# XuyangBai/D3Feat.pytorch

Measured on AMD Instinct MI355X. Metric: fragment-pairs/sec (fwd+bwd) on 3DMatch-shaped pairs, higher is better.
Workload: dtype f32

## Files before the change

### d3feat.pytorch_amd/_native.py

```python
import ctypes as C
import os
import subprocess

_PKG_DIR = os.path.dirname(os.path.abspath(__file__))
_REPO = os.path.dirname(_PKG_DIR)
LIB_PATH = os.path.join(_PKG_DIR, "libd3feat_hip.so")
CSRC = os.path.join(_PKG_DIR, "csrc")
SOURCES = ["radius_neighbors.hip", "grid_subsample.hip", "kpconv.hip", "kpconv_fused.hip", "kpconv_aggregate.hip", "kpconv_small.hip", "kpconv_deform.hip", "pool.hip", "detection.hip", "loss.hip",
           "reverse_table.hip", "kpconv_dx_gather.hip", "matching.hip", "elementwise.hip", "batchnorm.hip", "linear.hip", "gemm_epilogue.hip", "optimizer.hip", "misc.hip",
           "registration.hip", "nearest_pairs.hip", "icp.hip", "normals.hip", "augment.hip", "posegraph.hip", "tsdf.hip", "tsdf_integrate.hip", "tsdf_mesh.hip", "tsdf_sparse.hip", "odometry.hip", "tsdf_raycast.hip",
           "tsdf_mesh_sparse.hip"]

_vp, _i, _f, _sz = C.c_void_p, C.c_int, C.c_float, C.c_size_t
_d = C.c_double


class Tunables(C.Structure):
    _fields_ = [("atb_task_us", C.c_int32), ("atb_form", C.c_int32), ("atb_first_form_wgs", C.c_int32),
                ("match_wgs", C.c_int32), ("agg_through_lds", C.c_int32), ("atb_pipe", C.c_int32), ("xw_rows", C.c_int32), ("xw_split", C.c_int32),
                ("rowgemm_wide", C.c_int32), ("rowgemm_rt", C.c_int32), ("reserved", C.c_int32 * 6)]


class AtbProblem(C.Structure):
    _fields_ = [("x", _vp), ("grad_out", _vp), ("grad_w", _vp), ("N", C.c_int32), ("Cin", C.c_int32),
# ... 84 lines not shown
    "d3f_kpconv_packs_supports": (_i, [_i, _i, _i, _i, _i]),
    "d3f_kpconv_saves_wf": (_i, [_i, _i, _i, _i]),
    "d3f_kpconv_backward": (_i, [_vp, _i, _vp, _i, _vp, _i, _vp, _i, _vp, _i, _vp, _i, _f, _vp, _vp, _vp, _vp, _i,
                                 _vp, _vp, _vp, _sz, _vp]),
    "d3f_kpconv_grad_input_supported": (_i, [_i, _i, _i, _i]),
    "d3f_kpconv_aggregate": (_i, [_vp, _i, _vp, _i, _vp, _i, _vp, _i, _vp, _i, _f, _vp, _vp, _vp, _vp, _vp, _sz, _vp]),
    "d3f_kpconv_aggregate_modes": (_i, [_vp, _i, _vp, _i, _vp, _i, _vp, _i, _vp, _i, _f, _i, _vp, _vp, _vp]),
    "d3f_kpconv_grad_input_modes": (_i, [_vp, _i, _vp, _i, _vp, _i, _i, _vp, _i, _f, _i, _vp, _vp, _vp]),
    "d3f_kpconv_grad_input": (_i, [_vp, _i, _vp, _i, _vp, _i, _vp, _i, _vp, _i, _f, _vp, _vp, _i, _vp, _vp, _sz, _vp]),
    "d3f_kpconv_aggregate_transposed_supported": (_i, [_i, _i]),
    "d3f_kpconv_aggregate_transposed": (_i, [_vp, _i, _i, _i, _vp, _i, _f, _vp, _vp, _i, _vp, _vp]),
    "d3f_reverse_table_ws_bytes": (_sz, [_i, _i, _i]),
    "d3f_reverse_table_build": (_i, [_vp, _i, _i, _i, _vp, _vp, _vp, _sz, _vp]),
    "d3f_kpconv_grad_input_gather_supported": (_i, [_i, _i, _i]),
    "d3f_kpconv_grad_input_gather": (_i, [_vp, _i, _vp, _i, _vp, _vp, _vp, _i, _f, _vp, _vp, _i, _vp, _i, _i, _f, _vp, _vp, _vp,
                                          _vp, _vp]),
    "d3f_reverse_table_filter": (_i, [_vp, _i, _vp, _vp, _i, _vp, _i, _f, _vp, _vp, _vp]),
    "d3f_linear_grad_weight_supported": (_i, [_i, _i, _i]),
    "d3f_linear_fused_supported": (_i, [_i, _i, _i]),
    "d3f_linear_bias_act_forward": (_i, [_vp, _vp, _i, _i, _i, _vp, _vp, _vp, _f, _vp, _vp, _i, _vp]),
    "d3f_linear_pair_supported": (_i, [_i, _i, _i, _i]),
    "d3f_linear_pair_bias_act_forward": (_i, [_vp, _vp, _i, _vp, _vp, _i, _i, _i, _vp, _vp, _vp, _vp, _f, _vp, _vp, _i, _vp]),
    "d3f_linear_grad_input": (_i, [_vp, _vp, _i, _i, _i, _vp, _vp, _vp]),
    "d3f_linear_grad_weight_ws_bytes": (_sz, [_i, _i, _i]),
    "d3f_linear_grad_weight": (_i, [_vp, _vp, _i, _i, _i, _vp, _vp, _sz, _vp]),
    "d3f_linear_grad_weight_bias": (_i, [_vp, _vp, _i, _i, _i, _vp, _vp, _sz, _vp, _i, _i, _vp, _vp, _vp]),
    "d3f_permute_kpconv_weights": (_i, [_vp, _vp, _vp, _vp, _vp, _i, _vp]),
    "d3f_gemm_epilogue_supported": (_i, [_i, _i, _i, _i, _i]),
    "d3f_gemm_epilogue_ws_bytes": (_sz, [_i, _i, _i]),
    "d3f_gemm_epilogue": (_i, [_vp, _i, _vp, _i, _i, _i, _i, _i, _i, _vp, _vp, _vp, _i, _vp, _f, _vp, _i, _vp, _i, _vp, _sz,
                               _vp]),
    "d3f_bias_act_backward_blocks": (_i, [_i, _i]),
    "d3f_bias_act_backward_partial": (_i, [_vp, _vp, _f, _i, _i, _vp, _vp, _vp, _sz, _vp]),
    "d3f_bias_sum": (_i, [_vp, _i, _i, _vp, _vp, _vp]),
    "d3f_max_pool_forward": (_i, [_vp, _i, _i, _vp, _i, _i, _vp, _vp, _vp, _vp, _vp, _i, _i, _vp]),
    "d3f_max_pool_backward": (_i, [_vp, _vp, _i, _i, _i, _vp, _i, _vp]),
    "d3f_closest_pool_forward": (_i, [_vp, _i, _i, _vp, _i, _i, _vp, _i, _vp, _vp, _vp]),
    "d3f_closest_pool_backward": (_i, [_vp, _i, _vp, _i, _i, _i, _i, _vp, _i, _vp]),
    "d3f_bias_act_forward": (_i, [_vp, _vp, _vp, _vp, _f, _i, _i, _vp, _vp, _i, _vp, _vp, _i, _i, _vp]),
    "d3f_bias_act_backward_ws_bytes": (_sz, [_i, _i]),
    "d3f_bias_act_backward": (_i, [_vp, _vp, _f, _i, _i, _vp, _vp, _vp, _i, _vp, _vp, _sz, _vp]),
    "d3f_global_max": (_i, [_vp, _sz, _vp, _vp, _sz, _vp]),
    "d3f_global_max_rows": (_i, [_vp, _i, _i, _vp, _i, _vp, _vp, _sz, _vp]),
    "d3f_global_max_groups": (_i, [_vp, _i, _i, _vp, _i, _i, _vp, _vp, _sz, _vp]),
    "d3f_detection_scores_aux_floats": (_i, [_i]),
    "d3f_detection_scores_forward": (_i, [_vp, _i, _i, _vp, _i, _vp, _i, _vp, _vp, _vp, _vp, _i, _i, _vp]),
# ... 245 lines not shown
```

### d3feat.pytorch_amd/csrc/linear.hip

```cpp
#include <math.h>

#include <vector>

#include "kpconv_tile.hpp"

namespace d3f {

void* kpconv_timing_open(int which, hipStream_t stream, int Nq, int Ns, int H, int Cin, int Cout, int K);
void kpconv_timing_close(void* rec, hipStream_t stream);

template <int TI, int TJ, int U>
__global__ __launch_bounds__(256, 4) void atb_partial_kernel(const float* __restrict__ A, const float* __restrict__ B,
                                                             const float* __restrict__ row_div, int R, int M, int N,
                                                             int rows_per_wg, float* __restrict__ part) {
  typedef typename VecT<TI>::type VA;
  typedef typename VecT<TJ>::type VB;
  constexpr int HALVES = (TI * TJ >= 16) ? 2 : 1, TH = TI / HALVES;
  __shared__ float red[3][TH * TJ * 256];
  const int lane = threadIdx.x & 63, wave = threadIdx.x >> 6;
  const int li = lane & 15, lk = lane >> 4;
  const int nbj = N / (16 * TJ);
  const int m0 = (blockIdx.y / nbj) * 16 * TI, n0 = (blockIdx.y % nbj) * 16 * TJ;
  const int r0 = blockIdx.x * rows_per_wg, r1 = min(R, r0 + rows_per_wg);
  const float* ap = A + m0 + TI * li;
// ... 1059 lines not shown
bool rowgemm_pair_supported(int N, int K1, int K2, int M) {
  return N >= 4096 && ((M == 128 && K1 == 32 && K2 == 64) || (M == 64 && K1 == 16 && K2 == 32));
}

static int rowgemm_pair_launch(const float* X1, const float* W1, int K1, const float* X2, const float* W2, int K2, int N,
                               int M, const float* b1, const float* b2, const float* b3, const float* b4, float slope,
                               float* Y, float* zinit, int zn, hipStream_t stream) {
  if (!rowgemm_pair_supported(N, K1, K2, M)) return D3F_EINVAL;
  const int rw = tunables().rowgemm_wide;
  const bool wide = rw == 2 || (rw == 0 && N >= 65536);
#define D3F_RGPT(MBW, CS, KA, KB)                                                                                      \
  rowgemm_rt_kernel<MBW, CS, KA, KB><<<cdiv(N, 32 * (4 / CS)), 256, 0, stream>>>(X1, W1, X2, W2, N, b1, nullptr, b2, b3, \
                                                                                  b4, slope, Y, zinit, zn)
  if (M == 128) {
    if (wide) D3F_RGPT(4, 2, 2, 4); else D3F_RGPT(2, 4, 2, 4);
  } else {
    if (wide) D3F_RGPT(4, 1, 1, 2); else D3F_RGPT(2, 2, 1, 2);
  }
#undef D3F_RGPT
  D3F_LAUNCH_CHECK();
  return D3F_OK;
}

}

extern "C" {

int d3f_linear_grad_weight_supported(int N, int Cin, int Cout) { return d3f::atb_supported(N, Cout, Cin) ? 1 : 0; }

size_t d3f_linear_grad_weight_ws_bytes(int N, int Cin, int Cout) { return d3f::atb_ws_bytes(N, Cout, Cin); }

int d3f_linear_grad_weight(const float* x, const float* grad_out, int N, int Cin, int Cout, float* grad_w, void* ws,
                           size_t ws_bytes, void* stream) {
  if (!x || !grad_out || !grad_w || !ws || !d3f::atb_supported(N, Cout, Cin)) return D3F_EINVAL;
  if (ws_bytes < d3f::atb_ws_bytes(N, Cout, Cin)) return D3F_EWORKSPACE;
  return d3f::atb_splitk(grad_out, x, nullptr, N, Cout, Cin, grad_w, ws, (hipStream_t)stream);
}

int d3f_linear_grad_weight_bias(const float* x, const float* grad_out, int N, int Cin, int Cout, float* grad_w, void* ws,
                                size_t ws_bytes, const float* bias_part, int bias_blocks, int bias_cols,
                                float* grad_bias, float* grad_bias2, void* stream) {
  if (!x || !grad_out || !grad_w || !ws || !d3f::atb_supported(N, Cout, Cin)) return D3F_EINVAL;
  if (!bias_part || !grad_bias || bias_blocks < 1 || bias_cols < 1) return D3F_EINVAL;
  if (ws_bytes < d3f::atb_ws_bytes(N, Cout, Cin)) return D3F_EWORKSPACE;
  return d3f::atb_splitk_bias(grad_out, x, nullptr, N, Cout, Cin, grad_w, ws, (hipStream_t)stream, 0, bias_part,
                              bias_blocks, bias_cols, grad_bias, grad_bias2);
// ... 41 lines not shown
  return d3f::rowgemm_pair_supported(N, Cin1, Cin2, Cout) ? 1 : 0;
}

int d3f_linear_pair_bias_act_forward(const float* x1, const float* w1, int Cin1, const float* x2, const float* w2, int Cin2,
                                     int N, int Cout, const float* bias1, const float* bias2, const float* bias3,
                                     const float* bias4, float slope, float* out, float* zero_init, int zero_n,
                                     void* stream) {
  if (!x1 || !w1 || !x2 || !w2 || !out || !d3f::rowgemm_pair_supported(N, Cin1, Cin2, Cout) || (zero_init && zero_n < 1))
    return D3F_EINVAL;
  return d3f::rowgemm_pair_launch(x1, w1, Cin1, x2, w2, Cin2, N, Cout, bias1, bias2, bias3, bias4, slope, out, zero_init,
                                  zero_n, (hipStream_t)stream);
}

int d3f_linear_grad_input(const float* grad_out, const float* weight, int N, int Cin, int Cout, const float* add,
                          float* grad_x, void* stream) {
  if (!grad_out || !weight || !grad_x || !d3f::rowgemm_supported(N, Cout, Cin)) return D3F_EINVAL;
  if (add)
    return d3f::rowgemm_launch<false, true>(grad_out, weight, N, Cout, Cin, nullptr, add, nullptr, 1.0f, grad_x,
                                            nullptr, 0, (hipStream_t)stream);
  return d3f::rowgemm_launch<false, false>(grad_out, weight, N, Cout, Cin, nullptr, nullptr, nullptr, 1.0f, grad_x,
                                           nullptr, 0, (hipStream_t)stream);
}

}
```

### d3feat.pytorch_amd/ops.py

```python
import collections
import numpy as np
import ctypes
import threading

import torch

from . import _native

ORDER_REFERENCE = 0
ORDER_FIRST_SEEN = 1


def _stream():
    return torch.cuda.current_stream().cuda_stream


_PROFILER = None


def set_profiler(p):
    global _PROFILER
    _PROFILER = p


# ... 869 lines not shown
    def collect(self):
        self.closed = True
        g, self.tensor = self.tensor, None
        return g


class _GradTapFn(torch.autograd.Function):

    @staticmethod
    def forward(ctx, x, holder):
        ctx.holder = holder
        return x.view_as(x)

    @staticmethod
    def backward(ctx, g):
        return (None if ctx.holder.deposit(g) else g), None


def grad_tap(x, holder):
    return _GradTapFn.apply(x, holder) if holder is not None else x


def _add_deposited(holder, go, weight):
    c = holder.collect() if holder is not None else None
    if c is None:
        return torch.mm(go, weight)
    if c.is_contiguous() and c.dtype == go.dtype and c.shape == (go.shape[0], weight.shape[1]):
        if _WG_GROUP is not None:
            N, Cout, Cin = int(go.shape[0]), int(go.shape[1]), int(weight.shape[1])
            L = _native.lib()
            if go.is_contiguous() and weight.is_contiguous() and L.d3f_linear_fused_supported(N, Cin, Cout):
                gx = torch.empty_like(c)
                _native.check(L.d3f_linear_grad_input(_p(go), _p(weight), N, Cin, Cout, _p(c), _p(gx), _stream()),
                              "d3f_linear_grad_input")
                return gx
            return torch.addmm(c, go, weight)
        return c.addmm_(go, weight)
    return torch.mm(go, weight).add_(c)


GEMM_NT, GEMM_NN = 0, 1


def _al16(*ts):
    return all(t is None or t.data_ptr() % 16 == 0 for t in ts)


# ... 68 lines not shown
                                     b2 is not None and ctx.needs_input_grad[4], Cout, x.device)
        with _region("linear_fused_fwd[N=%d,Cin=%d,Cout=%d]" % (N, Cin, Cout), 4 * N * (Cin + Cout) + 4 * Cin * Cout):
            _native.check(L.d3f_linear_bias_act_forward(_p(x), _p(weight), N, Cin, Cout, _p(b1), _p(add), _p(b2),
                                                        float(slope), _p(out), _p(gbuf), nb * Cout, _stream()),
                          "d3f_linear_bias_act_forward")
        ctx.save_for_backward(x, weight, out)
        ctx.gbuf = gbuf
        ctx.gw_slot = _grad_slot(weight)
        ctx.slope = float(slope)
        ctx.has = (b1 is not None, add is not None, b2 is not None)
        return out

    @staticmethod
    def backward(ctx, grad_out):
        x, weight, out = ctx.saved_tensors
        L = _native.lib()
        N, Cin, Cout = int(x.shape[0]), int(x.shape[1]), int(weight.shape[0])
        go = grad_out.contiguous()
        want1 = ctx.has[0] and ctx.needs_input_grad[2]
        want2 = ctx.has[2] and ctx.needs_input_grad[4]
        g1, g2, first, second, pre = _bias_grad_rows(ctx, want1, want2, Cout, go.device)
        atb = ctx.needs_input_grad[1] and bool(L.d3f_linear_grad_weight_supported(N, Cin, Cout))
        bias_part, bias_blocks = None, 0
        if ctx.slope == 1.0 and not (want1 or want2):
            gm = go
        else:
            gm = go if ctx.slope == 1.0 else torch.empty_like(go)
            bias_part, bias_blocks = _epilogue_backward(go, out, ctx.slope, N, Cout, gm if ctx.slope != 1.0 else None,
                                                        first, second, pre, None, atb)
        gx = gw = None
        if ctx.needs_input_grad[0]:
            gx = torch.empty_like(x)
            c = ctx.holder.collect() if ctx.holder is not None else None
            if c is not None and not (c.is_contiguous() and c.shape == gx.shape and c.dtype == gx.dtype):
                c = c.contiguous().float().reshape(gx.shape)
            with _region("linear_dx[N=%d,Cin=%d,Cout=%d]" % (N, Cin, Cout), 4 * N * (Cin + Cout) + 4 * Cin * Cout):
                _native.check(L.d3f_linear_grad_input(_p(gm), _p(weight), N, Cin, Cout, _p(c), _p(gx), _stream()),
                              "d3f_linear_grad_input")
            if ctx.dep is not None and ctx.dep.deposit(gx):
                gx = None
        if ctx.needs_input_grad[1]:
            gw = _grad_target(ctx.gw_slot, weight)
            _weight_grad(x, gm, N, Cin, Cout, gw, atb, bias_part, bias_blocks, first, second)
        return (gx, _adoptable(gw, ctx.gw_slot), g1, gm if ctx.has[1] and ctx.needs_input_grad[3] else None, g2,
                None, None, None)


class _LinearPairBiasActFn(torch.autograd.Function):

    @staticmethod
    def forward(ctx, x1, w1, b1a, b1b, x2, w2, b2a, b2b, slope, deposit2=None):
        L = _native.lib()
        ctx.dep2 = deposit2
        N, C1, C2, Cout = int(x1.shape[0]), int(x1.shape[1]), int(x2.shape[1]), int(w1.shape[0])
        out = torch.empty((N, Cout), dtype=torch.float32, device=x1.device)
        ctx.want = tuple(b is not None and ctx.needs_input_grad[i] for b, i in ((b1a, 2), (b1b, 3), (b2a, 6), (b2b, 7)))
        gbuf, nb = _bias_grad_buffer(any(ctx.want), any(ctx.want), Cout, x1.device)
        with _region("linear_pair_fwd[N=%d,Cin=%d|%d,Cout=%d]" % (N, C1, C2, Cout),
                     4 * N * (C1 + C2 + Cout) + 4 * (C1 + C2) * Cout):
            _native.check(L.d3f_linear_pair_bias_act_forward(_p(x1), _p(w1), C1, _p(x2), _p(w2), C2, N, Cout, _p(b1a),
                                                             _p(b1b), _p(b2a), _p(b2b), float(slope), _p(out), _p(gbuf),
                                                             nb * Cout, _stream()), "d3f_linear_pair_bias_act_forward")
        ctx.save_for_backward(x1, w1, x2, w2, out)
        ctx.gbuf, ctx.slope = gbuf, float(slope)
        ctx.slots = (_grad_slot(w1), _grad_slot(w2))
        return out

    @staticmethod
    def backward(ctx, grad_out):
        x1, w1, x2, w2, out = ctx.saved_tensors
        L = _native.lib()
        N, C1, C2, Cout = int(x1.shape[0]), int(x1.shape[1]), int(x2.shape[1]), int(w1.shape[0])
        go = grad_out.contiguous()
        first, second, _, _, pre = _bias_grad_rows(ctx, any(ctx.want), any(ctx.want), Cout, go.device)
        need_w1, need_w2 = ctx.needs_input_grad[1], ctx.needs_input_grad[5]
        fold = need_w1 and need_w2 and _WG_GROUP is not None
        gm = torch.empty_like(go) if ctx.slope != 1.0 else go
        bias_part, bias_blocks = None, 0
        if ctx.slope != 1.0 or first is not None:
            bias_part, bias_blocks = _epilogue_backward(go, out, ctx.slope, N, Cout, gm if ctx.slope != 1.0 else None, first,
                                                        second, pre, None, fold and first is not None)
        third = fourth = None
        if first is not None:
            third, fourth = torch.empty_like(first), torch.empty_like(first)
        gx1 = gx2 = None
        if ctx.needs_input_grad[0]:
            gx1 = torch.empty_like(x1)
            _native.check(L.d3f_linear_grad_input(_p(gm), _p(w1), N, C1, Cout, None, _p(gx1), _stream()),
                          "d3f_linear_grad_input")
        if ctx.needs_input_grad[4]:
            gx2 = torch.empty_like(x2)
            _native.check(L.d3f_linear_grad_input(_p(gm), _p(w2), N, C2, Cout, None, _p(gx2), _stream()),
                          "d3f_linear_grad_input")
            if ctx.dep2 is not None and ctx.dep2.deposit(gx2):
                gx2 = None
        gw1 = gw2 = None
        if need_w1:
            gw1 = _grad_target(ctx.slots[0], w1)
            _weight_grad(x1, gm, N, C1, Cout, gw1, True, bias_part, bias_blocks, first, second)
        if need_w2:
            gw2 = _grad_target(ctx.slots[1], w2)
            _weight_grad(x2, gm, N, C2, Cout, gw2, True, bias_part, bias_blocks, third, fourth)
        if first is not None and bias_part is None:
            third.copy_(first)
            fourth.copy_(first)
        g = [first if ctx.want[0] else None, second if ctx.want[1] else None, third if ctx.want[2] else None,
             fourth if ctx.want[3] else None]
        return (gx1, _adoptable(gw1, ctx.slots[0]), g[0], g[1], gx2, _adoptable(gw2, ctx.slots[1]), g[2], g[3],
                None, None)


def linear_pair_supported(N, C1, C2, Cout, *tensors):
    for t in tensors:
        if not (t.is_cuda and t.dtype == torch.float32 and t.is_contiguous() and t.data_ptr() % 16 == 0):
            return False
    L = _native.lib()
    N, C1, C2, Cout = int(N), int(C1), int(C2), int(Cout)
    return bool(L.d3f_linear_pair_supported(N, C1, C2, Cout)) and bool(L.d3f_linear_fused_supported(N, C1, Cout)) \
        and bool(L.d3f_linear_fused_supported(N, C2, Cout))


def linear_pair_bias_act(x1, w1, b1a, b1b, x2, w2, b2a, b2b, slope=0.1, grad_deposit2=None):
    f = _opt_f32
    if not linear_pair_supported(x1.shape[0], x1.shape[1], x2.shape[1], w1.shape[0], x1, x2, w1, w2):
        raise RuntimeError("linear_pair_bias_act: unsupported operands x1%s x2%s w1%s w2%s" % (
            tuple(x1.shape), tuple(x2.shape), tuple(w1.shape), tuple(w2.shape)))
    return _LinearPairBiasActFn.apply(_f32(x1, "x1"), _f32(w1, "w1"), f(b1a, "bias"), f(b1b, "bias"), _f32(x2, "x2"),
                                      _f32(w2, "w2"), f(b2a, "bias"), f(b2b, "bias"), float(slope), grad_deposit2)


def _epilogue_backward(go, out, slope, N, C, gm, first, second, pre, row_div, fold):
    L = _native.lib()
# ... 141 lines not shown
            ctx.set_materialize_grads(False)
            return out, spack, gx_clear
        _native.check(L.d3f_bias_act_forward(_p(raw), _p(b1), _p(add), _p(b2), float(slope), N, C, _p(out), _p(gbuf),
                                             nb * C, None, None, 0, 0, _stream()), "d3f_bias_act_forward")
        ctx.save_for_backward(x, weight, out)
        return out

    @staticmethod
    def backward(ctx, grad_out, *_unused):
        x, weight, out = ctx.saved_tensors
        none = (None,) * 9
        if grad_out is None:
            return none
        L = _native.lib()
        N, Cin, Cout = int(x.shape[0]), int(x.shape[1]), int(weight.shape[0])
        go = grad_out.contiguous()
        want1 = ctx.has[0] and ctx.needs_input_grad[2]
        want2 = ctx.has[2] and ctx.needs_input_grad[4]
        g1, g2, first, second, pre = _bias_grad_rows(ctx, want1, want2, Cout, go.device)
        need_w = ctx.needs_input_grad[1]
        atb = need_w and N >= _SPLITK_MIN_ROWS and bool(L.d3f_linear_grad_weight_supported(N, Cin, Cout))
        bias_part, bias_blocks = None, 0
        identity = ctx.slope == 1.0
        if identity and first is None:
            gm = go
        else:
            gm = go if identity else torch.empty_like(go)
            bias_part, bias_blocks = _epilogue_backward(go, out, ctx.slope, N, Cout, None if identity else gm, first,
                                                        second, pre, None, atb)
        gx = _add_deposited(ctx.holder, gm, weight) if ctx.needs_input_grad[0] else None
        if gx is not None and ctx.dep is not None and ctx.dep.deposit(gx):
            gx = None
        gw = None
        if need_w:
            gw = _grad_target(ctx.gw_slot, weight)
            _weight_grad(x, gm, N, Cin, Cout, gw, atb, bias_part, bias_blocks, first, second)
        return (gx, _adoptable(gw, ctx.gw_slot), g1, gm if ctx.has[1] and ctx.needs_input_grad[3] else None, g2,
                None, None, None, None)


class _UpsampleLinearFn(torch.autograd.Function):

    @staticmethod
    def forward(ctx, xc, idx, skip, weight, b1, b2, slope, skip_deposit=None):
        L = _native.lib()
        ctx.skip_dep = skip_deposit
        Nc, Cc = int(xc.shape[0]), int(xc.shape[1])
        N, Cs = int(skip.shape[0]), int(skip.shape[1])
        Cout, H = int(weight.shape[0]), int(idx.shape[1])
        w1, w2 = weight[:, :Cc], weight[:, Cc:]
        t = torch.mm(xc, w1.t())
        y = torch.mm(skip, w2.t())
        out = torch.empty_like(y)
# ... 3866 lines not shown
```

### include/d3feat_hip.h

```cpp
#ifndef D3FEAT_HIP_H_
#define D3FEAT_HIP_H_

#include <stddef.h>
#include <stdint.h>

#ifdef __cplusplus
extern "C" {
#endif

#define D3F_OK 0
#define D3F_EINVAL (-1)
#define D3F_EWORKSPACE (-2)
#define D3F_ELAUNCH (-3)

#define D3F_ST_CAND_OVERFLOW 1
#define D3F_ST_CELL_RANGE 2
#define D3F_ST_TABLE_FULL 4
#define D3F_ST_CAPACITY 8
#define D3F_ST_WIDE_OVERFLOW 16
#define D3F_ST_NO_NEAREST 32

const char* d3f_version(void);
int d3f_device_arch_ok(void);
int d3f_device_arch_name(char* out, int n);
// ... 93 lines not shown
                         float* nn_out, void* spack_keep, float* grad_x_clear, void* ws, size_t ws_bytes,
                         void* stream);
int d3f_kpconv_grad_input(const float* q_pts, int Nq, const float* s_pts, int Ns, const int32_t* idx, int H,
                          const float* x, int Cin, const float* kernel_points, int K, float extent, const float* gwf,
                          const void* spack_kept, int grad_x_precleared, float* grad_x, void* ws, size_t ws_bytes,
                          void* stream);
int d3f_kpconv_aggregate_transposed_supported(int Cout, int K);
int d3f_kpconv_aggregate_transposed(const float* rev_rel, int rev_width, int Ns, int Nq, const float* kernel_points,
                                    int K, float extent, const float* nn, const float* grad_out, int Cout,
                                    float* agg_out, void* stream);

int d3f_linear_grad_weight_supported(int N, int Cin, int Cout);
int d3f_linear_fused_supported(int N, int Cin, int Cout);
int d3f_linear_bias_act_forward(const float* x, const float* weight, int N, int Cin, int Cout, const float* bias1,
                                const float* add, const float* bias2, float slope, float* out, float* zero_init,
                                int zero_n, void* stream);
int d3f_linear_pair_supported(int N, int Cin1, int Cin2, int Cout);
int d3f_linear_pair_bias_act_forward(const float* x1, const float* w1, int Cin1, const float* x2, const float* w2, int Cin2,
                                     int N, int Cout, const float* bias1, const float* bias2, const float* bias3,
                                     const float* bias4, float slope, float* out, float* zero_init, int zero_n,
                                     void* stream);
int d3f_linear_grad_input(const float* grad_out, const float* weight, int N, int Cin, int Cout, const float* add,
                          float* grad_x, void* stream);
int d3f_permute_kpconv_weights(const float* const* srcs_host, float* const* dsts_host, const int* K_host,
                               const int* Cin_host, const int* Cout_host, int n, void* stream);
int d3f_gemm_epilogue_supported(int R, int K, int N, int mode, int kblock);
size_t d3f_gemm_epilogue_ws_bytes(int R, int K, int N);
int d3f_gemm_epilogue(const float* x, int ldx, const float* w, int ldw, int mode, int kblock, int R, int K, int N,
                      const float* row_div, const float* bias1, const float* add, int ldadd, const float* bias2,
                      float slope, float* y, int ldy, float* zero_init, int zero_n, void* ws, size_t ws_bytes,
                      void* stream);
size_t d3f_linear_grad_weight_ws_bytes(int N, int Cin, int Cout);
int d3f_linear_grad_weight(const float* x, const float* grad_out, int N, int Cin, int Cout, float* grad_w, void* ws,
                           size_t ws_bytes, void* stream);
int d3f_linear_grad_weight_bias(const float* x, const float* grad_out, int N, int Cin, int Cout, float* grad_w, void* ws,
                                size_t ws_bytes, const float* bias_part, int bias_blocks, int bias_cols,
                                float* grad_bias, float* grad_bias2, void* stream);
typedef struct d3f_atb_problem {
  const float* x;
  const float* grad_out;
  float* grad_w;
  int32_t N, Cin, Cout, ldw;
  const float* bias_part;
  int32_t bias_blocks, bias_cols;
  float* grad_bias;
  float* grad_bias2;
// ... 595 lines not shown
```

### profiles/rowgemm_bench.py

```python
import os
import sys

import numpy as np
import torch

sys.path.insert(0, os.path.dirname(os.path.dirname(os.path.abspath(__file__))))
from d3feat_pytorch_amd import _native


def graph_timed(fn, reps=20):
    fn()
    torch.cuda.synchronize()
    s = torch.cuda.Stream()
    g = torch.cuda.CUDAGraph()
    with torch.cuda.stream(s):
        fn()
        s.synchronize()
        with torch.cuda.graph(g, stream=s):
            for _ in range(reps):
                fn()
    torch.cuda.synchronize()
    g.replay()
    torch.cuda.synchronize()
    e0, e1 = torch.cuda.Event(enable_timing=True), torch.cuda.Event(enable_timing=True)
# ... 58 lines not shown
        sc = torch.empty((N, M), device="cuda")
        y = torch.empty((N, M), device="cuda")
        y2 = torch.empty((N, M), device="cuda")

        def two():
            st = torch.cuda.current_stream().cuda_stream
            _native.check(L.d3f_linear_bias_act_forward(x2.data_ptr(), w2.data_ptr(), N, K2, M, b[2].data_ptr(), None,
                                                        b[3].data_ptr(), 1.0, sc.data_ptr(), None, 0, st), "sc")
            _native.check(L.d3f_linear_bias_act_forward(x1.data_ptr(), w1.data_ptr(), N, K1, M, b[0].data_ptr(), sc.data_ptr(),
                                                        b[1].data_ptr(), 0.1, y.data_ptr(), None, 0, st), "u2")

        def one():
            st = torch.cuda.current_stream().cuda_stream
            _native.check(L.d3f_linear_pair_bias_act_forward(x1.data_ptr(), w1.data_ptr(), K1, x2.data_ptr(), w2.data_ptr(), K2,
                                                             N, M, b[0].data_ptr(), b[1].data_ptr(), b[2].data_ptr(),
                                                             b[3].data_ptr(), 0.1, y2.data_ptr(), None, 0, st), "pair")
        t2, t1 = graph_timed(two), graph_timed(one)
        two()
        one()
        err = float((y - y2).abs().max() / y.abs().max())
        print("%-34s %10.1f %10.1f   rel diff %.1e" % ("%d x (%d | %d) -> %d" % (N, K1, K2, M), t2, t1, err))


if __name__ == "__main__" and len(sys.argv) > 1 and sys.argv[1] == "pair":
    pair()
if __name__ == "__main__" and len(sys.argv) == 1:
    main()
```

Measured before the change: 719.6.

## Fuse leaky-ReLU mask, bias-grad partials and grad-input GEMM into one kernel

Adds a row-GEMM MFMA kernel that applies the leaky-ReLU backward mask to grad_out on the fly, optionally writes the masked gradient, accumulates per-block bias-gradient partials via DPP row reductions, and computes grad_input plus the residual add in a single launch. A pair variant produces both grad inputs for the two-weight linear. The Python backward paths use it by default when shapes and alignment allow. This removes a separate mask/bias kernel and a re-read of the masked gradient, at the cost of more complex kernels and extra register pressure.

```diff
diff --git a/d3feat.pytorch_amd/_native.py b/d3feat.pytorch_amd/_native.py
--- a/d3feat.pytorch_amd/_native.py
+++ b/d3feat.pytorch_amd/_native.py
@@ -130,6 +130,12 @@
     "d3f_linear_pair_supported": (_i, [_i, _i, _i, _i]),
     "d3f_linear_pair_bias_act_forward": (_i, [_vp, _vp, _i, _vp, _vp, _i, _i, _i, _vp, _vp, _vp, _vp, _f, _vp, _vp, _i, _vp]),
     "d3f_linear_grad_input": (_i, [_vp, _vp, _i, _i, _i, _vp, _vp, _vp]),
+    "d3f_linear_grad_input_act_supported": (_i, [_i, _i, _i]),
+    "d3f_linear_grad_input_act_blocks": (_i, [_i, _i]),
+    "d3f_linear_grad_input_act_ws_bytes": (_sz, [_i, _i]),
+    "d3f_linear_grad_input_act": (_i, [_vp, _vp, _f, _vp, _i, _i, _i, _vp, _vp, _vp, _vp, _sz, _vp]),
+    "d3f_linear_pair_grad_input_act_supported": (_i, [_i, _i, _i, _i]),
+    "d3f_linear_pair_grad_input_act": (_i, [_vp, _vp, _f, _vp, _i, _vp, _i, _i, _i, _vp, _vp, _vp, _vp, _sz, _vp]),
     "d3f_linear_grad_weight_ws_bytes": (_sz, [_i, _i, _i]),
     "d3f_linear_grad_weight": (_i, [_vp, _vp, _i, _i, _i, _vp, _vp, _sz, _vp]),
     "d3f_linear_grad_weight_bias": (_i, [_vp, _vp, _i, _i, _i, _vp, _vp, _sz, _vp, _i, _i, _vp, _vp, _vp]),
diff --git a/d3feat.pytorch_amd/csrc/linear.hip b/d3feat.pytorch_amd/csrc/linear.hip
--- a/d3feat.pytorch_amd/csrc/linear.hip
+++ b/d3feat.pytorch_amd/csrc/linear.hip
@@ -1105,6 +1105,226 @@
   return D3F_OK;
 }
 
+template <int CTRL>
+__device__ __forceinline__ float dpp_rot(float v) {
+  return __int_as_float(__builtin_amdgcn_update_dpp(0, __float_as_int(v), CTRL, 0xF, 0xF, false));
+}
+__device__ __forceinline__ float row16_sum(float v) {
+  v += dpp_rot<0x128>(v);
+  v += dpp_rot<0x124>(v);
+  v += dpp_rot<0x122>(v);
+  v += dpp_rot<0x121>(v);
+  return v;
+}
+
+template <int MB>
+__device__ __forceinline__ void vstore(float* dst, const float (&v)[MB]) {
+  if constexpr (MB == 4) *(float4*)dst = make_float4(v[0], v[MB > 1 ? 1 : 0], v[MB > 2 ? 2 : 0], v[MB > 3 ? 3 : 0]);
+  else if constexpr (MB == 2) *(float2*)dst = make_float2(v[0], v[MB > 1 ? 1 : 0]);
+  else dst[0] = v[0];
+}
+
+template <int MB1, int MB2, int CS, int BT, int KT>
+__global__ __launch_bounds__(256) void rowgemm_act_kernel(const float* __restrict__ go, const float* __restrict__ out,
+                                                          float slope, const float* __restrict__ W1,
+                                                          const float* __restrict__ W2, int N,
+                                                          const float* __restrict__ add, float* __restrict__ Y1,
+                                                          float* __restrict__ Y2, float* __restrict__ gm,
+                                                          float* __restrict__ part) {
+  constexpr int M1 = 16 * MB1 * CS, M2 = 16 * MB2 * CS, TPP = 4 / CS, B2 = MB2 > 0 ? MB2 : 1;
+  constexpr int P = BT == 4 ? CS : 1;
+  constexpr int K = 16 * KT, D = KT < 4 ? KT : 4;
+  typedef typename VecT<MB1>::type V1;
+  typedef typename VecT<B2>::type V2;
+  __shared__ float4 sb[4][64];
+  const int lane = threadIdx.x & 63, wave = threadIdx.x >> 6;
+  const int li = lane & 15, lk = lane >> 4;
+  const int cg = wave % CS, ts = wave / CS;
+  const int cb1 = cg * 16 * MB1 + MB1 * li, cb2 = cg * 16 * MB2 + MB2 * li;
+  const bool masked = slope != 1.0f;
+  const int ntiles = (N + 15) / 16;
+  float4 bsum = make_float4(0.f, 0.f, 0.f, 0.f);
+#pragma unroll
+  for (int p = 0; p < P; ++p) {
+    const int row0 = (blockIdx.x * TPP * P + p * TPP + ts) * 16;
+    if (row0 >= N) continue;
+    const bool live = row0 + li < N;
+    const size_t off = (size_t)min(row0 + li, N - 1) * K + 4 * lk;
+    f32x4 acc1[MB1], acc2[B2];
+#pragma unroll
+    for (int n = 0; n < MB1; ++n) acc1[n] = (f32x4){0.f, 0.f, 0.f, 0.f};
+#pragma unroll
+    for (int n = 0; n < B2; ++n) acc2[n] = (f32x4){0.f, 0.f, 0.f, 0.f};
+    struct AFrag { float4 a, o; };
+    struct BFrag { float b1[MB1][4], b2[B2][4]; };
+    auto load_a = [&](AFrag& f, int kt) {
+      f.a = *(const float4*)(go + off + 16 * kt);
+      if (masked) f.o = *(const float4*)(out + off + 16 * kt);
+    };
+    auto load_b = [&](BFrag& f, int kt) {
+#pragma unroll
+      for (int t = 0; t < 4; ++t) {
+        const V1 wv = *(const V1*)(W1 + (size_t)(16 * kt + 4 * lk + t) * M1 + cb1);
+#pragma unroll
+        for (int n = 0; n < MB1; ++n) f.b1[n][t] = vget<MB1>(wv, n);
+        if constexpr (MB2 > 0) {
+          const V2 wu = *(const V2*)(W2 + (size_t)(16 * kt + 4 * lk + t) * M2 + cb2);
+#pragma unroll
+          for (int n = 0; n < B2; ++n) f.b2[n][t] = vget<B2>(wu, n);
+        }
+      }
+    };
+    auto step = [&](const AFrag& fa, const BFrag& f, int kt) {
+      float4 a = fa.a;
+      if (masked) {
+        a.x = a.x * (fa.o.x > 0.0f ? 1.0f : slope);
+        a.y = a.y * (fa.o.y > 0.0f ? 1.0f : slope);
+        a.z = a.z * (fa.o.z > 0.0f ? 1.0f : slope);
+        a.w = a.w * (fa.o.w > 0.0f ? 1.0f : slope);
+      }
+      if (kt % CS == cg) {
+        if (gm && live) *(float4*)(gm + (size_t)(row0 + li) * K + 16 * kt + 4 * lk) = a;
+        if (part) {
+          const float4 z = live ? a : make_float4(0.f, 0.f, 0.f, 0.f);
+          const float sx = row16_sum(z.x), sy = row16_sum(z.y), sz = row16_sum(z.z), sw = row16_sum(z.w);
+          if (li == kt) { bsum.x += sx; bsum.y += sy; bsum.z += sz; bsum.w += sw; }
+        }
+      }
+#pragma unroll
+      for (int n = 0; n < MB1; ++n) {
+        acc1[n] = __builtin_amdgcn_mfma_f32_16x16x4f32(a.x, f.b1[n][0], acc1[n], 0, 0, 0);
+        acc1[n] = __builtin_amdgcn_mfma_f32_16x16x4f32(a.y, f.b1[n][1], acc1[n], 0, 0, 0);
+        acc1[n] = __builtin_amdgcn_mfma_f32_16x16x4f32(a.z, f.b1[n][2], acc1[n], 0, 0, 0);
+        acc1[n] = __builtin_amdgcn_mfma_f32_16x16x4f32(a.w, f.b1[n][3], acc1[n], 0, 0, 0);
+      }
+      if constexpr (MB2 > 0) {
+#pragma unroll
+        for (int n = 0; n < B2; ++n) {
+          acc2[n] = __builtin_amdgcn_mfma_f32_16x16x4f32(a.x, f.b2[n][0], acc2[n], 0, 0, 0);
+          acc2[n] = __builtin_amdgcn_mfma_f32_16x16x4f32(a.y, f.b2[n][1], acc2[n], 0, 0, 0);
+          acc2[n] = __builtin_amdgcn_mfma_f32_16x16x4f32(a.z, f.b2[n][2], acc2[n], 0, 0, 0);
+          acc2[n] = __builtin_amdgcn_mfma_f32_16x16x4f32(a.w, f.b2[n][3], acc2[n], 0, 0, 0);
+        }
+      }
+    };
+    AFrag fa[KT];
+    BFrag fb[2];
+    load_b(fb[0], 0);
+#pragma unroll
+    for (int d = 0; d < D; ++d) load_a(fa[d], d);
+#pragma unroll
+    for (int kt = 0; kt < KT; ++kt) {
+      if (kt + 1 < KT) load_b(fb[(kt + 1) & 1], kt + 1);
+      if (kt + D < KT) load_a(fa[kt + D], kt + D);
+      step(fa[kt], fb[kt & 1], kt);
+    }
+#pragma unroll
+    for (int r = 0; r < 4; ++r) {
+      const int row = row0 + 4 * lk + r;
+      if (row < N) {
+        float v[MB1];
+#pragma unroll
+        for (int n = 0; n < MB1; ++n) v[n] = acc1[n][r];
+        if (add) {
+          const V1 av = *(const V1*)(add + (size_t)row * M1 + cb1);
+#pragma unroll
+          for (int n = 0; n < MB1; ++n) v[n] += vget<MB1>(av, n);
+        }
+        vstore<MB1>(Y1 + (size_t)row * M1 + cb1, v);
+        if constexpr (MB2 > 0) {
+          float u[B2];
+#pragma unroll
+          for (int n = 0; n < B2; ++n) u[n] = acc2[n][r];
+          vstore<B2>(Y2 + (size_t)row * M2 + cb2, u);
+        }
+      }
+    }
+  }
+  if (!part) return;
+  sb[wave][4 * li + lk] = bsum;
+  __syncthreads();
+  if constexpr (BT == 4) {
+    if ((int)threadIdx.x < K / 4) {
+      const float4 s0 = sb[0][threadIdx.x], s1 = sb[1][threadIdx.x], s2 = sb[2][threadIdx.x], s3 = sb[3][threadIdx.x];
+      *(float4*)(part + (size_t)blockIdx.x * K + 4 * threadIdx.x) =
+          make_float4((s0.x + s1.x) + (s2.x + s3.x), (s0.y + s1.y) + (s2.y + s3.y), (s0.z + s1.z) + (s2.z + s3.z),
+                      (s0.w + s1.w) + (s2.w + s3.w));
+    }
+  } else {
+    const int s = threadIdx.x >> 6, t = threadIdx.x & 63;
+    const int tile = blockIdx.x * TPP + s;
+    if (s < TPP && t < K / 4 && tile < ntiles) {
+      float4 v = sb[s * CS][t];
+#pragma unroll
+      for (int w = 1; w < CS; ++w) {
+        const float4 u = sb[s * CS + w][t];
+        v.x += u.x; v.y += u.y; v.z += u.z; v.w += u.w;
+      }
+      *(float4*)(part + (size_t)tile * K + 4 * t) = v;
+    }
+  }
+}
+
+static bool act_dim(int c) { return c == 32 || c == 64 || c == 128 || c == 256; }
+
+bool rowgemm_act_supported(int N, int K, int M) { return N >= 4096 && act_dim(K) && act_dim(M); }
+
+bool rowgemm_act_pair_supported(int N, int K, int M1, int M2) {
+  return N >= 4096 && ((K == 128 && M1 == 32 && M2 == 64) || (K == 64 && M1 == 16 && M2 == 32));
+}
+
+static int act_block_rows(int N) { return N >= 65536 ? 64 : 16; }
+int rowgemm_act_blocks(int N) { return cdiv(N, act_block_rows(N)); }
+
+static int rowgemm_act_launch(const float* go, const float* out, float slope, const float* W, int N, int K, int M,
+                              const float* add, float* Y, float* gm, float* part, hipStream_t stream) {
+  const int rw = tunables().rowgemm_wide;
+  const bool wide = rw == 2 || (rw == 0 && N >= 65536);
+  const bool b64 = act_block_rows(N) == 64;
+#define D3F_RGA2(MBW, CS, KT)                                                                                          \
+  do {                                                                                                                 \
+    if (b64)                                                                                                           \
+      rowgemm_act_kernel<MBW, 0, CS, 4, KT><<<cdiv(N, 64), 256, 0, stream>>>(go, out, slope, W, nullptr, N, add, Y,    \
+                                                                            nullptr, gm, part);                       \
+    else                                                                                                               \
+      rowgemm_act_kernel<MBW, 0, CS, 1, KT><<<cdiv(N, 16 * (4 / CS)), 256, 0, stream>>>(go, out, slope, W, nullptr, N, \
+                                                                                       add, Y, nullptr, gm, part);    \
+  } while (0)
+#define D3F_RGA(MBW, CS)                  \
+  do {                                    \
+    if (K == 32) D3F_RGA2(MBW, CS, 2);    \
+    else if (K == 64) D3F_RGA2(MBW, CS, 4);  \
+    else if (K == 128) D3F_RGA2(MBW, CS, 8); \
+    else D3F_RGA2(MBW, CS, 16);           \
+  } while (0)
+  switch (M) {
+    case 32: D3F_RGA(1, 2); break;
+    case 64: if (wide) D3F_RGA(4, 1); else D3F_RGA(2, 2); break;
+    case 128: if (wide) D3F_RGA(4, 2); else D3F_RGA(2, 4); break;
+    case 256: D3F_RGA(4, 4); break;
+    default: return D3F_EINVAL;
+  }
+#undef D3F_RGA
+#undef D3F_RGA2
+  D3F_LAUNCH_CHECK();
+  return D3F_OK;
+}
+
+static int rowgemm_act_pair_launch(const float* go, const float* out, float slope, const float* W1, const float* W2,
+                                   int N, int K, float* Y1, float* Y2, float* gm, float* part, hipStream_t stream) {
+  const bool b64 = act_block_rows(N) == 64;
+#define D3F_RGAP(MB1, MB2, BT, KT) \
+  rowgemm_act_kernel<MB1, MB2, 1, BT, KT><<<cdiv(N, 64), 256, 0, stream>>>(go, out, slope, W1, W2, N, nullptr, Y1, Y2, gm, part)
+  if (K == 128) {
+    if (b64) D3F_RGAP(2, 4, 4, 8); else D3F_RGAP(2, 4, 1, 8);
+  } else {
+    if (b64) D3F_RGAP(1, 2, 4, 4); else D3F_RGAP(1, 2, 1, 4);
+  }
+#undef D3F_RGAP
+  D3F_LAUNCH_CHECK();
+  return D3F_OK;
+}
+
 }
 
 extern "C" {
@@ -1192,4 +1412,50 @@
                                            nullptr, 0, (hipStream_t)stream);
 }
 
-}
+int d3f_linear_grad_input_act_supported(int N, int Cin, int Cout) {
+  return d3f::rowgemm_act_supported(N, Cout, Cin) ? 1 : 0;
+}
+
+int d3f_linear_pair_grad_input_act_supported(int N, int Cin1, int Cin2, int Cout) {
+  return d3f::rowgemm_act_pair_supported(N, Cout, Cin1, Cin2) ? 1 : 0;
+}
+
+int d3f_linear_grad_input_act_blocks(int N, int Cout) {
+  return (N >= 4096 && Cout >= 1) ? d3f::rowgemm_act_blocks(N) : 0;
+}
+
+size_t d3f_linear_grad_input_act_ws_bytes(int N, int Cout) {
+  const int blocks = d3f_linear_grad_input_act_blocks(N, Cout);
+  return blocks ? d3f::align_up(sizeof(float) * (size_t)blocks * (size_t)Cout, 256) : 0;
+}
+
+static bool act_args_ok(const float* grad_out, const float* out, float slope, const float* grad_masked,
+                        const float* bias_part, size_t ws_bytes, int N, int Cout) {
+  if (!grad_out || !out || (!grad_masked && slope != 1.0f)) return false;
+  if ((((uintptr_t)grad_out | (uintptr_t)out | (uintptr_t)grad_masked | (uintptr_t)bias_part) & 15) != 0) return false;
+  return !bias_part || ws_bytes >= d3f_linear_grad_input_act_ws_bytes(N, Cout);
+}
+
+int d3f_linear_grad_input_act(const float* grad_out, const float* out, float slope, const float* weight, int N, int Cin,
+                              int Cout, const float* add, float* grad_x, float* grad_masked, float* bias_part,
+                              size_t ws_bytes, void* stream) {
+  if (!weight || !grad_x || !d3f::rowgemm_act_supported(N, Cout, Cin) ||
+      !act_args_ok(grad_out, out, slope, grad_masked, bias_part, ws_bytes, N, Cout) ||
+      (((uintptr_t)weight | (uintptr_t)add | (uintptr_t)grad_x) & 15) != 0)
+    return D3F_EINVAL;
+  return d3f::rowgemm_act_launch(grad_out, out, slope, weight, N, Cout, Cin, add, grad_x, grad_masked, bias_part,
+                                 (hipStream_t)stream);
+}
+
+int d3f_linear_pair_grad_input_act(const float* grad_out, const float* out, float slope, const float* w1, int Cin1,
+                                   const float* w2, int Cin2, int N, int Cout, float* grad_x1, float* grad_x2,
+                                   float* grad_masked, float* bias_part, size_t ws_bytes, void* stream) {
+  if (!w1 || !w2 || !grad_x1 || !grad_x2 || !d3f::rowgemm_act_pair_supported(N, Cout, Cin1, Cin2) ||
+      !act_args_ok(grad_out, out, slope, grad_masked, bias_part, ws_bytes, N, Cout) ||
+      (((uintptr_t)w1 | (uintptr_t)w2 | (uintptr_t)grad_x1 | (uintptr_t)grad_x2) & 15) != 0)
+    return D3F_EINVAL;
+  return d3f::rowgemm_act_pair_launch(grad_out, out, slope, w1, w2, N, Cout, grad_x1, grad_x2, grad_masked, bias_part,
+                                      (hipStream_t)stream);
+}
+
+}
diff --git a/d3feat.pytorch_amd/ops.py b/d3feat.pytorch_amd/ops.py
--- a/d3feat.pytorch_amd/ops.py
+++ b/d3feat.pytorch_amd/ops.py
@@ -915,7 +915,15 @@
 
 
 def _add_deposited(holder, go, weight):
-    c = holder.collect() if holder is not None else None
+    return _add_collected(holder.collect() if holder is not None else None, go, weight)
+
+
+def _deposit_streams(c, N, Cin, Cout, weight):
+    return c is not None and _WG_GROUP is not None and c.is_contiguous() and c.dtype == torch.float32 and \
+        c.shape == (N, Cin) and weight.is_contiguous() and bool(_native.lib().d3f_linear_fused_supported(N, Cin, Cout))
+
+
+def _add_collected(c, go, weight):
     if c is None:
         return torch.mm(go, weight)
     if c.is_contiguous() and c.dtype == go.dtype and c.shape == (go.shape[0], weight.shape[1]):
@@ -1030,21 +1038,34 @@
         g1, g2, first, second, pre = _bias_grad_rows(ctx, want1, want2, Cout, go.device)
         atb = ctx.needs_input_grad[1] and bool(L.d3f_linear_grad_weight_supported(N, Cin, Cout))
         bias_part, bias_blocks = None, 0
-        if ctx.slope == 1.0 and not (want1 or want2):
+        identity = ctx.slope == 1.0 and not (want1 or want2)
+        gx = gw = c = None
+        if ctx.needs_input_grad[0]:
+            gx = torch.empty_like(x)
+            c = ctx.holder.collect() if ctx.holder is not None else None
+            if c is not None and not (c.is_contiguous() and c.shape == gx.shape and c.dtype == gx.dtype):
+                c = c.contiguous().float().reshape(gx.shape)
+        fused = _FUSED_GRAD_INPUT_ACT and gx is not None and atb and not identity and \
+            bool(L.d3f_linear_grad_input_act_supported(N, Cin, Cout)) and _aligned16(go, out, weight, c, gx)
+        if fused:
+            gm = go if ctx.slope == 1.0 else torch.empty_like(go)
+            bias_part, nws, bias_blocks = _grad_input_act_ws(N, Cout, go.device, first is not None)
+            with _region("linear_dx_act[N=%d,Cin=%d,Cout=%d]" % (N, Cin, Cout),
+                         4 * N * (Cin + 3 * Cout) + 4 * Cin * Cout):
+                _native.check(L.d3f_linear_grad_input_act(_p(go), _p(out), ctx.slope, _p(weight), N, Cin, Cout, _p(c),
+                                                          _p(gx), _p(gm) if ctx.slope != 1.0 else None, _p(bias_part),
+                                                          nws, _stream()), "d3f_linear_grad_input_act")
+        elif identity:
             gm = go
         else:
             gm = go if ctx.slope == 1.0 else torch.empty_like(go)
             bias_part, bias_blocks = _epilogue_backward(go, out, ctx.slope, N, Cout, gm if ctx.slope != 1.0 else None,
                                                         first, second, pre, None, atb)
-        gx = gw = None
-        if ctx.needs_input_grad[0]:
-            gx = torch.empty_like(x)
-            c = ctx.holder.collect() if ctx.holder is not None else None
-            if c is not None and not (c.is_contiguous() and c.shape == gx.shape and c.dtype == gx.dtype):
-                c = c.contiguous().float().reshape(gx.shape)
-            with _region("linear_dx[N=%d,Cin=%d,Cout=%d]" % (N, Cin, Cout), 4 * N * (Cin + Cout) + 4 * Cin * Cout):
-                _native.check(L.d3f_linear_grad_input(_p(gm), _p(weight), N, Cin, Cout, _p(c), _p(gx), _stream()),
-                              "d3f_linear_grad_input")
+        if gx is not None:
+            if not fused:
+                with _region("linear_dx[N=%d,Cin=%d,Cout=%d]" % (N, Cin, Cout), 4 * N * (Cin + Cout) + 4 * Cin * Cout):
+                    _native.check(L.d3f_linear_grad_input(_p(gm), _p(weight), N, Cin, Cout, _p(c), _p(gx), _stream()),
+                                  "d3f_linear_grad_input")
             if ctx.dep is not None and ctx.dep.deposit(gx):
                 gx = None
         if ctx.needs_input_grad[1]:
@@ -1085,21 +1106,36 @@
         fold = need_w1 and need_w2 and _WG_GROUP is not None
         gm = torch.empty_like(go) if ctx.slope != 1.0 else go
         bias_part, bias_blocks = None, 0
-        if ctx.slope != 1.0 or first is not None:
-            bias_part, bias_blocks = _epilogue_backward(go, out, ctx.slope, N, Cout, gm if ctx.slope != 1.0 else None, first,
-                                                        second, pre, None, fold and first is not None)
         third = fourth = None
         if first is not None:
             third, fourth = torch.empty_like(first), torch.empty_like(first)
-        gx1 = gx2 = None
-        if ctx.needs_input_grad[0]:
-            gx1 = torch.empty_like(x1)
+        gx1 = torch.empty_like(x1) if ctx.needs_input_grad[0] else None
+        gx2 = torch.empty_like(x2) if ctx.needs_input_grad[4] else None
+        fused = _FUSED_GRAD_INPUT_ACT and gx1 is not None and gx2 is not None and need_w1 and need_w2 and \
+            (ctx.slope != 1.0 or first is not None) and \
+            bool(L.d3f_linear_pair_grad_input_act_supported(N, C1, C2, Cout)) and _aligned16(go, out, w1, w2, gx1, gx2)
+        if fused:
+            part, nws, blocks = _grad_input_act_ws(N, Cout, go.device, first is not None)
+            with _region("linear_pair_dx_act[N=%d,Cin=%d|%d,Cout=%d]" % (N, C1, C2, Cout),
+                         4 * N * (C1 + C2 + 3 * Cout) + 4 * (C1 + C2) * Cout):
+                _native.check(L.d3f_linear_pair_grad_input_act(_p(go), _p(out), ctx.slope, _p(w1), C1, _p(w2), C2, N, Cout,
+                                                               _p(gx1), _p(gx2), _p(gm) if ctx.slope != 1.0 else None,
+                                                               _p(part), nws, _stream()),
+                              "d3f_linear_pair_grad_input_act")
+            if part is not None and fold:
+                bias_part, bias_blocks = part, blocks
+            elif part is not None:
+                _native.check(L.d3f_bias_sum(_p(part), blocks, Cout, _p(first), _p(second), _stream()), "d3f_bias_sum")
+        elif ctx.slope != 1.0 or first is not None:
+            bias_part, bias_blocks = _epilogue_backward(go, out, ctx.slope, N, Cout, gm if ctx.slope != 1.0 else None, first,
+                                                        second, pre, None, fold and first is not None)
+        if gx1 is not None and not fused:
             _native.check(L.d3f_linear_grad_input(_p(gm), _p(w1), N, C1, Cout, None, _p(gx1), _stream()),
                           "d3f_linear_grad_input")
-        if ctx.needs_input_grad[4]:
-            gx2 = torch.empty_like(x2)
-            _native.check(L.d3f_linear_grad_input(_p(gm), _p(w2), N, C2, Cout, None, _p(gx2), _stream()),
-                          "d3f_linear_grad_input")
+        if gx2 is not None:
+            if not fused:
+                _native.check(L.d3f_linear_grad_input(_p(gm), _p(w2), N, C2, Cout, None, _p(gx2), _stream()),
+                              "d3f_linear_grad_input")
             if ctx.dep2 is not None and ctx.dep2.deposit(gx2):
                 gx2 = None
         gw1 = gw2 = None
@@ -1116,6 +1152,21 @@
              fourth if ctx.want[3] else None]
         return (gx1, _adoptable(gw1, ctx.slots[0]), g[0], g[1], gx2, _adoptable(gw2, ctx.slots[1]), g[2], g[3],
                 None, None)
+
+
+_FUSED_GRAD_INPUT_ACT = True
+
+
+def _aligned16(*tensors):
+    return all(t is None or t.data_ptr() % 16 == 0 for t in tensors)
+
+
+def _grad_input_act_ws(N, C, device, want):
+    if not want:
+        return None, 0, 0
+    L = _native.lib()
+    nbytes = int(L.d3f_linear_grad_input_act_ws_bytes(N, C))
+    return _ws(nbytes, device), nbytes, int(L.d3f_linear_grad_input_act_blocks(N, C))
 
 
 def linear_pair_supported(N, C1, C2, Cout, *tensors):
@@ -1303,13 +1354,24 @@
         atb = need_w and N >= _SPLITK_MIN_ROWS and bool(L.d3f_linear_grad_weight_supported(N, Cin, Cout))
         bias_part, bias_blocks = None, 0
         identity = ctx.slope == 1.0
+        c = ctx.holder.collect() if ctx.needs_input_grad[0] and ctx.holder is not None else None
+        gx = None
         if identity and first is None:
             gm = go
         else:
             gm = go if identity else torch.empty_like(go)
-            bias_part, bias_blocks = _epilogue_backward(go, out, ctx.slope, N, Cout, None if identity else gm, first,
-                                                        second, pre, None, atb)
-        gx = _add_deposited(ctx.holder, gm, weight) if ctx.needs_input_grad[0] else None
+            if _FUSED_GRAD_INPUT_ACT and atb and go.is_contiguous() and _deposit_streams(c, N, Cin, Cout, weight) and \
+                    bool(L.d3f_linear_grad_input_act_supported(N, Cin, Cout)) and _aligned16(go, out, weight, c):
+                gx = torch.empty_like(c)
+                bias_part, nws, bias_blocks = _grad_input_act_ws(N, Cout, go.device, first is not None)
+                _native.check(L.d3f_linear_grad_input_act(_p(go), _p(out), ctx.slope, _p(weight), N, Cin, Cout, _p(c),
+                                                          _p(gx), None if identity else _p(gm), _p(bias_part), nws,
+                                                          _stream()), "d3f_linear_grad_input_act")
+            else:
+                bias_part, bias_blocks = _epilogue_backward(go, out, ctx.slope, N, Cout, None if identity else gm, first,
+                                                            second, pre, None, atb)
+        if gx is None and ctx.needs_input_grad[0]:
+            gx = _add_collected(c, gm, weight)
         if gx is not None and ctx.dep is not None and ctx.dep.deposit(gx):
             gx = None
         gw = None
diff --git a/include/d3feat_hip.h b/include/d3feat_hip.h
--- a/include/d3feat_hip.h
+++ b/include/d3feat_hip.h
@@ -139,6 +139,16 @@
                                      void* stream);
 int d3f_linear_grad_input(const float* grad_out, const float* weight, int N, int Cin, int Cout, const float* add,
                           float* grad_x, void* stream);
+int d3f_linear_grad_input_act_supported(int N, int Cin, int Cout);
+int d3f_linear_grad_input_act_blocks(int N, int Cout);
+size_t d3f_linear_grad_input_act_ws_bytes(int N, int Cout);
+int d3f_linear_grad_input_act(const float* grad_out, const float* out, float slope, const float* weight, int N, int Cin,
+                              int Cout, const float* add, float* grad_x, float* grad_masked, float* bias_part,
+                              size_t ws_bytes, void* stream);
+int d3f_linear_pair_grad_input_act_supported(int N, int Cin1, int Cin2, int Cout);
+int d3f_linear_pair_grad_input_act(const float* grad_out, const float* out, float slope, const float* w1, int Cin1,
+                                   const float* w2, int Cin2, int N, int Cout, float* grad_x1, float* grad_x2,
+                                   float* grad_masked, float* bias_part, size_t ws_bytes, void* stream);
 int d3f_permute_kpconv_weights(const float* const* srcs_host, float* const* dsts_host, const int* K_host,
                                const int* Cin_host, const int* Cout_host, int n, void* stream);
 int d3f_gemm_epilogue_supported(int R, int K, int N, int mode, int kblock);
diff --git a/profiles/rowgemm_bench.py b/profiles/rowgemm_bench.py
--- a/profiles/rowgemm_bench.py
+++ b/profiles/rowgemm_bench.py
@@ -104,6 +104,61 @@
         print("%-34s %10.1f %10.1f   rel diff %.1e" % ("%d x (%d | %d) -> %d" % (N, K1, K2, M), t2, t1, err))
 
 
+ACT_NODES = [(6208, 128, 256, True), (6208, 256, 64, False), (23808, 64, 256, True), (23808, 256, 64, False),
+             (23808, 64, 256, True), (23808, 256, 64, False), (23808, 64, 128, True), (23808, 128, 32, False),
+             (114624, 32, 128, True), (114624, 128, (32, 64), False), (114624, 32, 64, True)]
+
+
+def act():
+    L = _native.lib()
+    rng = np.random.default_rng(2)
+    print("%-34s %10s %10s   %s" % ("node (rows x Cout -> Cin)", "parent us", "one us", "GB/s of the one launch (go + out + gm + add + gx)"))
+    tot = [0.0, 0.0]
+    for (N, Cout, Cin, res) in ACT_NODES:
+        cins = Cin if isinstance(Cin, tuple) else (Cin,)
+        mk = lambda *s: torch.from_numpy(rng.normal(size=s).astype(np.float32)).cuda()
+        go, out = mk(N, Cout), mk(N, Cout)
+        ws_ = [mk(Cout, c) for c in cins]
+        add = mk(N, cins[0]) if res else None
+        gm, gm2 = torch.empty_like(go), torch.empty_like(go)
+        gxs, gxs2 = [torch.empty((N, c), device="cuda") for c in cins], [torch.empty((N, c), device="cuda") for c in cins]
+        nws = int(L.d3f_bias_act_backward_ws_bytes(N, Cout))
+        part = torch.empty(nws, dtype=torch.uint8, device="cuda")
+        nws2 = int(L.d3f_linear_grad_input_act_ws_bytes(N, Cout))
+        part2 = torch.empty(nws2, dtype=torch.uint8, device="cuda")
+        p = lambda t: t.data_ptr() if t is not None else None
+
+        def parent():
+            st = torch.cuda.current_stream().cuda_stream
+            _native.check(L.d3f_bias_act_backward_partial(p(go), p(out), 0.1, N, Cout, p(gm), None, p(part), nws, st), "mask")
+            for w, c, gx in zip(ws_, cins, gxs):
+                _native.check(L.d3f_linear_grad_input(p(gm), p(w), N, c, Cout, p(add), p(gx), st), "dx")
+
+        def one():
+            st = torch.cuda.current_stream().cuda_stream
+            if len(cins) == 1:
+                _native.check(L.d3f_linear_grad_input_act(p(go), p(out), 0.1, p(ws_[0]), N, cins[0], Cout, p(add), p(gxs2[0]),
+                                                          p(gm2), p(part2), nws2, st), "dx_act")
+            else:
+                _native.check(L.d3f_linear_pair_grad_input_act(p(go), p(out), 0.1, p(ws_[0]), cins[0], p(ws_[1]), cins[1], N,
+                                                               Cout, p(gxs2[0]), p(gxs2[1]), p(gm2), p(part2), nws2, st),
+                              "pair_dx_act")
+        t0, t1 = graph_timed(parent), graph_timed(one)
+        parent()
+        one()
+        torch.cuda.synchronize()
+        same = torch.equal(gm, gm2) and all(torch.equal(a, b) for a, b in zip(gxs, gxs2))
+        nbytes = 4.0 * N * (3 * Cout + sum(cins) * (2 if res else 1))
+        print("%-34s %10.1f %10.1f   %5.0f   %s" % (
+            "%d x %d -> %s%s" % (N, Cout, "|".join(str(c) for c in cins), " + add" if res else ""), t0, t1,
+            nbytes / t1 * 1e-3, "bit-identical" if same else "DIFFERENT"))
+        tot[0] += t0
+        tot[1] += t1
+    print("%-34s %10.1f %10.1f" % ("sum of the eleven nodes", tot[0], tot[1]))
+
+
+if __name__ == "__main__" and len(sys.argv) > 1 and sys.argv[1] == "act":
+    act()
 if __name__ == "__main__" and len(sys.argv) > 1 and sys.argv[1] == "pair":
     pair()
 if __name__ == "__main__" and len(sys.argv) == 1:
```

Result: no change. 712.8 (-0.9%).
